# AutoGPTQ/AutoGPTQ

Hardware: AMD Instinct MI355X
Metric: int4 g128 QuantLinear fwd GB/s + tokens/s, Llama-7B shapes (higher is better)
Workload: dtype f16; 1 GPU; Llama-7B linear shapes (4096->4096 x4, 4096->11008 x2, 11008->4096) x 32 blocks = 224 layers, int4 g128 no act-order, M=1 rows per step, 128 launches/step in one hipGraph (q|k|v and gate|up of a block: one gptq_forward_multi launch each); layers=224, launches=128, parallelism=single

## Files before the change

### autogptq_amd/csrc/gemv_tiled_kernel.cuh

```cuda
#pragma once
#include <cstddef>

#include "gemv_shared.cuh"

namespace gptq {

struct TiledSeg {
    const void* bias;
    void* out;
    int N, col0;
};
struct PeerEpi {
    char* xbuf[2][GPTQ_PEER_MAX];
    unsigned* flags[GPTQ_PEER_MAX];
    unsigned* state;
    int world, rank;
    unsigned row_bytes, col_off_bytes, owners, pad_;
};
struct TiledParams {
    int blk_end[4];
    const void* x;
    int M, K;
    int chunks, chunks_per_split, ksplit, gu_shift, groups, xstride, waves;
    int pair_strips;
    const unsigned* tq[4];
    const void* cst[4];
    const int* perm[4];
    int xraw_off;
    int nseg, nsum;
    unsigned max_spins;
    TiledSeg seg[4];
    unsigned long long* gran;
    unsigned* epochs;
    unsigned* err;
    PeerEpi peer;
};
static_assert(offsetof(TiledParams, perm) == 128, "the entry batch of the decode-copy kernel is the first two cache lines of its arguments");

template <int BITS> struct TiledFmt;
template <> struct TiledFmt<4> { static constexpr int WPL = 4, KPL = 32, REC = 48, ZB = 1; };
template <> struct TiledFmt<8> { static constexpr int WPL = 4, KPL = 16, REC = 64, ZB = 2; };
template <> struct TiledFmt<3> { static constexpr int WPL = 3, KPL = 32, REC = 48, ZB = 1; };
template <> struct TiledFmt<2> { static constexpr int WPL = 2, KPL = 32, REC = 48, ZB = 1; };

#ifdef GPTQ_TILED_STAMPS
#define TILED_STAMP(i) (st_[i] = __builtin_amdgcn_s_memtime() | vz_)
#define TILED_STAMPS_OUT() stamps_out()
#define TILED_HOT_END() return
#else
#define TILED_HOT_END() __builtin_amdgcn_endpgm()
#define TILED_STAMP(i) ((void)0)
#define TILED_STAMPS_OUT() ((void)0)
#endif

template <int N_> struct WordsOf { typedef unsigned type __attribute__((ext_vector_type(N_))); };

template <int BITS, int MT, int U, typename T, int MAXW, int XM = 0, int ZM2 = 0>
__global__ void __launch_bounds__(MAXW * 64, MAXW == 16 ? 4 : 2) gemv_tiled_kernel(TiledParams p) {
#ifdef GPTQ_TILED_STAMPS
    unsigned long long st_[9] = {};
    unsigned vz_;
    asm volatile("v_mov_b32 %0, 0" : "=v"(vz_));
    st_[7] = __builtin_amdgcn_s_memrealtime() | vz_;
    TILED_STAMP(0);
    auto stamps_out = [&]() {
        st_[8] = __builtin_amdgcn_s_memrealtime() | vz_;
        unsigned long long* const dbg = p.gran;
        const int b = (int)blockIdx.x, nb = (int)gridDim.x;
        const int slot = b == 0 ? 0 : (b == 1 ? 1 : (b == nb / 2 ? 2 : (b == nb - 1 ? 3 : -1)));
        if (dbg != nullptr && p.ksplit == 1 && slot >= 0 && (threadIdx.x & 63) == 0) {
#pragma unroll
            for (int i = 0; i < 9; ++i) dbg[(slot * 16 + (int)(threadIdx.x >> 6)) * 16 + i] = st_[i];
        }
    };
#endif
    constexpr bool BF = std::is_same_v<T, bf16>;
    constexpr bool ACT = XM == 1, PEER = XM == 3;
    constexpr bool PAIR = XM == 4;
    constexpr bool MULTI = XM == 5 || XM == 6;
    constexpr int NSTR = PAIR ? 2 : (XM == 5 ? 4 : (XM == 6 ? 2 : 1));
    using F = TiledFmt<BITS>;
    constexpr int WPL = F::WPL, KPL = F::KPL, CKE = 4 * KPL, CHB = 64 * WPL * 4, REC = F::REC, NX = KPL / 8;
    constexpr int LKPL = KPL == 32 ? 5 : 4;
    typedef typename WordsOf<WPL>::type qvec;
    unsigned m_lo, m_hi, m_b, magic;
    asm("s_mov_b32 %0, 0x000f000f" : "=s"(m_lo));
    asm("s_mov_b32 %0, 0x00f000f0" : "=s"(m_hi));
    asm("s_mov_b32 %0, 0x00ff00ff" : "=s"(m_b));
    asm("v_mov_b32 %0, 0x64006400" : "=v"(magic));
    unsigned m2a, m2b, m2c, m2d, m2e;
    asm("s_mov_b32 %0, 0x00030003" : "=s"(m2a));
    asm("s_mov_b32 %0, 0x000c000c" : "=s"(m2b));
    asm("s_mov_b32 %0, 0x00300030" : "=s"(m2c));
    asm("s_mov_b32 %0, 0x00c000c0" : "=s"(m2d));
    asm("s_mov_b32 %0, 0x03000300" : "=s"(m2e));
    unsigned m3a, m3b, m3c;
    asm("s_mov_b32 %0, 0x00070007" : "=s"(m3a));
    asm("s_mov_b32 %0, 0x00380038" : "=s"(m3b));
    asm("s_mov_b32 %0, 0x01c001c0" : "=s"(m3c));
    extern __shared__ __attribute__((aligned(16))) char smem[];
    const int tid = threadIdx.x, lane = tid & 63;
    const int wave = __builtin_amdgcn_readfirstlane(tid >> 6);
    const int col = lane & 15, kb = lane >> 4;
    typedef unsigned u32x16 __attribute__((ext_vector_type(16)));
    typedef unsigned long long u64x8 __attribute__((ext_vector_type(8)));
    typedef unsigned long long u64x4 __attribute__((ext_vector_type(4)));
    static_assert(offsetof(TiledParams, x) == 16 && offsetof(TiledParams, M) == 24 && offsetof(TiledParams, chunks) == 32 && offsetof(TiledParams, pair_strips) == 60 &&
                  offsetof(TiledParams, tq) == 64 && offsetof(TiledParams, cst) == 96 && offsetof(TiledParams, perm) == 128 && offsetof(TiledParams, xraw_off) == 160, "the entry batch");
    u32x16 ha;
    u64x8 hb;
    [[maybe_unused]] u64x4 hp = {};
    [[maybe_unused]] int xraw_off = 0;
    {
        const auto kargs = __builtin_amdgcn_kernarg_segment_ptr();
        if constexpr (ACT)
            asm volatile("s_load_dwordx16 %0, %4, 0x0\n\ts_load_dwordx16 %1, %4, 0x40\n\ts_load_dwordx8 %2, %4, 0x80\n\ts_load_dword %3, %4, 0xa0\n\ts_waitcnt lgkmcnt(0)"
                         : "=&s"(ha), "=&s"(hb), "=&s"(hp), "=&s"(xraw_off) : "s"(kargs));
        else
            asm volatile("s_load_dwordx16 %0, %2, 0x0\n\ts_load_dwordx16 %1, %2, 0x40\n\ts_waitcnt lgkmcnt(0)" : "=&s"(ha), "=&s"(hb) : "s"(kargs));
    }
    const int be0 = (int)ha[0], be1 = (int)ha[1], be2 = (int)ha[2], Mrows = (int)ha[6], K = (int)ha[7], nchunks = (int)ha[8], cps = (int)ha[9], ksplit = (int)ha[10],
              gshift = (int)ha[11], G = (int)ha[12], xstride = (int)ha[13], W = (int)ha[14];
    [[maybe_unused]] const int hstrips = (int)ha[15];
    typedef __attribute__((address_space(1))) const char gchar;
    gchar* const xg = (gchar*)(((unsigned long long)ha[5] << 32) | ha[4]);
    int sidx = blockIdx.x, ks = 0, cb = 0, ce = nchunks, kbeg = 0, kend = K;
    if (__builtin_expect(ksplit != 1, 0)) {
        sidx = (int)blockIdx.x / ksplit; ks = (int)blockIdx.x - sidx * ksplit;
        cb = ks * cps; ce = min(cb + cps, nchunks);
        kbeg = cb * CKE; kend = min(ce * CKE, K);
    }
    unsigned long long tqs_ = hb[0], csts_ = hb[4];
    [[maybe_unused]] unsigned long long perm_ = hp[0];
    int sbase = 0, s = 0;
    if constexpr (ACT)
        asm("s_cmp_ge_i32 %[i], %[e0]\n\ts_cbranch_scc0 1f\n\t"
            "s_mov_b64 %[tq], %[tq1]\n\ts_mov_b64 %[cs], %[cs1]\n\ts_mov_b64 %[pm], %[pm1]\n\ts_mov_b32 %[sb], %[e0]\n\ts_mov_b32 %[s], 1\n\t"
            "s_cmp_ge_i32 %[i], %[e1]\n\ts_cselect_b64 %[tq], %[tq2], %[tq]\n\ts_cselect_b64 %[cs], %[cs2], %[cs]\n\ts_cselect_b64 %[pm], %[pm2], %[pm]\n\ts_cselect_b32 %[sb], %[e1], %[sb]\n\ts_cselect_b32 %[s], 2, %[s]\n\t"
            "s_cmp_ge_i32 %[i], %[e2]\n\ts_cselect_b64 %[tq], %[tq3], %[tq]\n\ts_cselect_b64 %[cs], %[cs3], %[cs]\n\ts_cselect_b64 %[pm], %[pm3], %[pm]\n\ts_cselect_b32 %[sb], %[e2], %[sb]\n\ts_cselect_b32 %[s], 3, %[s]\n"
            "1:"
            : [tq] "+&s"(tqs_), [cs] "+&s"(csts_), [pm] "+&s"(perm_), [sb] "+&s"(sbase), [s] "+&s"(s)
            : [i] "s"(sidx), [e0] "s"(be0), [e1] "s"(be1), [e2] "s"(be2), [tq1] "s"(hb[1]), [tq2] "s"(hb[2]), [tq3] "s"(hb[3]), [cs1] "s"(hb[5]), [cs2] "s"(hb[6]), [cs3] "s"(hb[7]),
              [pm1] "s"(hp[1]), [pm2] "s"(hp[2]), [pm3] "s"(hp[3])
            : "scc");
    else
        asm("s_cmp_ge_i32 %[i], %[e0]\n\ts_cbranch_scc0 1f\n\t"
            "s_mov_b64 %[tq], %[tq1]\n\ts_mov_b64 %[cs], %[cs1]\n\ts_mov_b32 %[sb], %[e0]\n\ts_mov_b32 %[s], 1\n\t"
            "s_cmp_ge_i32 %[i], %[e1]\n\ts_cselect_b64 %[tq], %[tq2], %[tq]\n\ts_cselect_b64 %[cs], %[cs2], %[cs]\n\ts_cselect_b32 %[sb], %[e1], %[sb]\n\ts_cselect_b32 %[s], 2, %[s]\n\t"
            "s_cmp_ge_i32 %[i], %[e2]\n\ts_cselect_b64 %[tq], %[tq3], %[tq]\n\ts_cselect_b64 %[cs], %[cs3], %[cs]\n\ts_cselect_b32 %[sb], %[e2], %[sb]\n\ts_cselect_b32 %[s], 3, %[s]\n"
            "1:"
            : [tq] "+&s"(tqs_), [cs] "+&s"(csts_), [sb] "+&s"(sbase), [s] "+&s"(s)
            : [i] "s"(sidx), [e0] "s"(be0), [e1] "s"(be1), [e2] "s"(be2), [tq1] "s"(hb[1]), [tq2] "s"(hb[2]), [tq3] "s"(hb[3]), [cs1] "s"(hb[5]), [cs2] "s"(hb[6]), [cs3] "s"(hb[7])
            : "scc");
    gchar* const tqs = (gchar*)tqs_;
    gchar* const csts = (gchar*)csts_;
    [[maybe_unused]] const int* const permp = (const int*)perm_;
    const int strip = sidx - sbase;
    const int Wh = NSTR == 4 ? (W >> 2) : (NSTR == 2 ? (W >> 1) : W);
    const int sel = NSTR == 1 ? 0 : (scalar_ge(wave, Wh) + (NSTR == 4 ? scalar_ge(wave, 2 * Wh) + scalar_ge(wave, 3 * Wh) : 0));
    const int wv = NSTR == 1 ? wave : wave - sel * Wh;
    const int strip_w = PAIR ? strip + sel * hstrips : (MULTI ? strip * NSTR + sel : strip);
    char* const xs = smem;
    char* const cs = smem + (size_t)MT * xstride;
    const unsigned crec = (unsigned)G * (unsigned)REC;
    const size_t cpad = ((size_t)crec + 15) & ~(size_t)15;
    float* const red = (float*)(cs + NSTR * cpad);
    gchar* const tb = tqs + (size_t)(unsigned)strip_w * ((unsigned)nchunks * (unsigned)CHB);
    gchar* const cg = csts + (size_t)(unsigned)(MULTI ? strip * NSTR : strip) * crec;
    const unsigned t_lane = (unsigned)lane * (WPL * 4u);
    auto stage_all = [&]() __attribute__((always_inline)) {
        const unsigned xs_lds = (unsigned)(size_t)(__attribute__((address_space(3))) char*)xs, cs_lds = (unsigned)(size_t)(__attribute__((address_space(3))) char*)cs;
        const int w64 = wave * 64, step = W * 64;
        gchar* xrow[MT];
        unsigned xdst[MT];
        if constexpr (XM == 0 || XM == 3 || XM == 4 || MULTI) {
#pragma unroll
            for (int m = 0; m < MT; ++m) {
                xrow[m] = xg + (unsigned)((m == 0 ? 0 : min(m, Mrows - 1)) * K + kbeg) * 2u;
                xdst[m] = xs_lds + m * xstride;
            }
            stage_rows<MT, false>(xrow, xdst, tid, w64, step, (kend - kbeg) >> 3);
        } else if constexpr (ACT) {
#pragma unroll
            for (int m = 0; m < MT; ++m) {
                xrow[m] = xg + (unsigned)((m == 0 ? 0 : min(m, Mrows - 1)) * K) * 2u;
                xdst[m] = xs_lds + (unsigned)xraw_off + m * (K * 2 + 16);
            }
            stage_rows<MT, false>(xrow, xdst, tid, w64, step, K >> 3);
        }
        const int cpieces = (int)(crec >> 4) * (MULTI ? NSTR : 1);
        if constexpr (PAIR) {
            gchar* const crow[2] = {cg, cg + (size_t)(unsigned)hstrips * crec};
            const unsigned cdst[2] = {cs_lds, cs_lds + (unsigned)cpad};
            stage_rows<2, true>(crow, cdst, tid, w64, step, cpieces);
        } else {
            gchar* const crow[1] = {cg};
            const unsigned cdst[1] = {cs_lds};
            stage_rows<1, true>(crow, cdst, tid, w64, step, cpieces);
        }
    };
#ifndef GPTQ_TILED_WEIGHTS_FIRST
    stage_all();
#endif
    typedef int i32x4 __attribute__((ext_vector_type(4)));
    i32x4 pa[2][2] = {};
    const int apieces = ACT ? (kend - kbeg) >> 3 : 0;
    if constexpr (ACT) {
        const int* const pg = permp + kbeg;
        if (tid < apieces) { pa[0][0] = *(const i32x4*)(pg + tid * 8); pa[0][1] = *(const i32x4*)(pg + tid * 8 + 4); }
        if (tid + W * 64 < apieces) { pa[1][0] = *(const i32x4*)(pg + (tid + W * 64) * 8); pa[1][1] = *(const i32x4*)(pg + (tid + W * 64) * 8 + 4); }
    }
    auto x_gather = [&]() {
        const int* const pg = permp + kbeg;
        const char* const xraw = smem + xraw_off;
        for (int pc0 = tid; pc0 < apieces; pc0 += 2 * W * 64) {
            const int pcb = pc0 + W * 64;
            const bool two = pcb < apieces;
            if (pc0 != tid) {
                pa[0][0] = *(const i32x4*)(pg + pc0 * 8); pa[0][1] = *(const i32x4*)(pg + pc0 * 8 + 4);
                if (two) { pa[1][0] = *(const i32x4*)(pg + pcb * 8); pa[1][1] = *(const i32x4*)(pg + pcb * 8 + 4); }
            }
#pragma unroll
            for (int m = 0; m < MT; ++m) {
                const unsigned short* xr = (const unsigned short*)(xraw + (size_t)m * (K * 2 + 16));
#pragma unroll
                for (int h = 0; h < 2; ++h) {
                    if (h == 1 && !two) break;
                    unsigned short v[8];
#pragma unroll
                    for (int i = 0; i < 8; ++i) v[i] = xr[pa[h][i >> 2][i & 3]];
                    u32x4 o;
#pragma unroll
                    for (int i = 0; i < 4; ++i) o[i] = (unsigned)v[2 * i] | ((unsigned)v[2 * i + 1] << 16);
                    *(u32x4*)(xs + (size_t)m * xstride + (size_t)(h ? pcb : pc0) * 16) = o;
                }
            }
        }
    };
#if defined(GPTQ_TILED_ZM)
    constexpr bool ZM = BITS == 4 && MT <= 4 && (GPTQ_TILED_ZM == 2 || (GPTQ_TILED_ZM == 1 && BF));
#else
    constexpr bool ZM = BITS == 4 && BF && (MT == 4 || (MT == 2 && ZM2 == 1));
#endif
#ifdef GPTQ_TILED_NO_XS
    constexpr bool XS = false;
#else
    constexpr bool XS = BF && BITS == 4 && MT <= 2 && !ZM;
#endif
    constexpr bool XC = BF && MT <= 2 && !XS && !ZM;
    using MM = std::conditional_t<XC, f16, T>;
    constexpr int ES = MT * 16 + 4;
    float* const xe = red + W * ES;
    auto x_to_f16 = [&]() {
        const int prow = (kend - kbeg) >> 3, total = prow * MT;
        for (int i0 = 0; i0 < total; i0 += W * 64) {
            const int idx = i0 + tid;
            const bool ok = idx < total;
            int m = 0, pc = ok ? idx : 0;
            if constexpr (MT > 1) { m = pc / prow; pc -= m * prow; }
            u32x4* const at = (u32x4*)(xs + (size_t)m * xstride + (size_t)pc * 16);
            u32x4 v = {0u, 0u, 0u, 0u};
            if (ok) v = *at;
            unsigned mx = 0u;
#pragma unroll
            for (int i = 0; i < 4; ++i) {
                const unsigned a = v[i] & 0x7fff7fffu;
                mx = max(mx, max(a & 0xffffu, a >> 16));
            }
            mx = max(mx, (unsigned)__shfl_xor((int)mx, 1, 64));
            if constexpr (NX == 4) mx = max(mx, (unsigned)__shfl_xor((int)mx, 2, 64));
            const int E = (int)((mx >> 7) & 0xffu);
            const int ms = min(max(268 - E, 1), 253);
            const float mult = __builtin_bit_cast(float, (unsigned)ms << 23);
#pragma unroll
            for (int i = 0; i < 4; ++i) {
                const float lo = __builtin_bit_cast(float, v[i] << 16) * mult, hi = __builtin_bit_cast(float, v[i] & 0xffff0000u) * mult;
                v[i] = __builtin_bit_cast(unsigned, __builtin_amdgcn_cvt_pkrtz(lo, hi));
            }
            if (ok) {
                *at = v;
                if ((pc & (NX - 1)) == 0) xe[(pc / NX) * 4 + m] = __builtin_bit_cast(float, (unsigned)(254 - ms) << 23);
            }
        }
        __syncthreads();
    };
    auto x_sums = [&]() {
        const int prow = (kend - kbeg) >> 3, total = prow * MT;
        for (int i0 = 0; i0 < total; i0 += W * 64) {
            const int idx = i0 + tid;
            const bool ok = idx < total;
            int m = 0, pc = ok ? idx : 0;
            if constexpr (MT > 1) { m = pc / prow; pc -= m * prow; }
            u32x4 v = {0u, 0u, 0u, 0u};
            if (ok) v = *(const u32x4*)(xs + (size_t)m * xstride + (size_t)pc * 16);
            float sm = 0.f;
#pragma unroll
            for (int i = 0; i < 4; ++i) sm += __builtin_bit_cast(float, v[i] << 16) + __builtin_bit_cast(float, v[i] & 0xffff0000u);
            sm += __shfl_xor(sm, 1, 64);
            if constexpr (NX == 4) sm += __shfl_xor(sm, 2, 64);
            if (ok && (pc & (NX - 1)) == 0) xe[(pc / NX) * 4 + m] = sm;
        }
        __syncthreads();
    };
    const char* const xl = xs + (size_t)min(lane & 3, MT - 1) * xstride + kb * (KPL * 2);
    const char* const xl2 = xs + (size_t)min(4 + (lane & 3), MT - 1) * xstride + kb * (KPL * 2);
    float acc[MT];
#pragma unroll
    for (int m = 0; m < MT; ++m) acc[m] = 0.f;
    const f16x2 k960 = {(f16)960.f, (f16)960.f}, k896 = {(f16)896.f, (f16)896.f}, k1008 = {(f16)1008.f, (f16)1008.f};
    const f16x2 r16 = {(f16)0.0625f, (f16)0.0625f}, r8 = {(f16)0.125f, (f16)0.125f}, r64 = {(f16)0.015625f, (f16)0.015625f};
    const f16x2 k768 = {(f16)768.f, (f16)768.f}, k1020 = {(f16)1020.f, (f16)1020.f}, r4 = {(f16)0.25f, (f16)0.25f}, r256 = {(f16)0.00390625f, (f16)0.00390625f};
    auto bits_of = [&](f16x2 hv) -> unsigned {
        if constexpr (BF && !XC) {
            const bf16x2 o = {(bf16)(float)hv[0], (bf16)(float)hv[1]};
            return __builtin_bit_cast(unsigned, o);
        } else {
            return __builtin_bit_cast(unsigned, hv);
        }
    };
    constexpr int E = MT * 16, NE = (MULTI ? NSTR : 1) * E;
    const int n_t = (MULTI ? strip * NSTR + tid / E : strip) * 16 + (tid & 15);
    float bv0 = 0.f, bv1 = 0.f;
    typedef __attribute__((address_space(1))) T gT;
    int N = 0;
    const void* biasp = nullptr;
    void* outp = nullptr;
    auto seg_request = [&]() __attribute__((always_inline)) {
        int sl = s;
        asm volatile("" : "+s"(sl) : : "memory");
        N = p.seg[sl].N; biasp = p.seg[sl].bias; outp = p.seg[sl].out;
    };
    auto seg_pin = [&]() __attribute__((always_inline)) { asm volatile("" : "+s"(N), "+s"(biasp), "+s"(outp)); };
    bool staged = false;
    for (int cbase = cb; cbase < ce; cbase += Wh * U) {
        const int c0 = cbase + wv * U;
        qvec q[U];
#pragma unroll
        for (int j = 0; j < U; ++j) q[j] = __builtin_nontemporal_load((const __attribute__((address_space(1))) qvec*)(tb + ((unsigned)min(c0 + j, ce - 1) * (unsigned)CHB + t_lane)));
        if (!staged) {
            TILED_STAMP(1);
            seg_request();
#ifdef GPTQ_TILED_WEIGHTS_FIRST
            stage_all();
            asm volatile("s_waitcnt vmcnt(0)" ::: "memory");
#else
            asm volatile("s_waitcnt vmcnt(%0)" ::"n"(U) : "memory");
#endif
            if constexpr (ACT) {
                __syncthreads();
                x_gather();
            }
            __syncthreads();
            if constexpr (XC) x_to_f16();
            if constexpr (XS) x_sums();
            seg_pin();
            if (biasp != nullptr && tid < NE && n_t < (PAIR ? N >> 1 : N)) {
                bv0 = DType<T>::to_f32(((const gT*)biasp)[n_t]);
                if constexpr (PAIR) bv1 = DType<T>::to_f32(((const gT*)biasp)[n_t + (N >> 1)]);
            }
            TILED_STAMP(2);
            staged = true;
        }
#ifdef GPTQ_TILED_STAMPS
        if (cbase + Wh * U >= ce) { asm volatile("s_waitcnt vmcnt(0)" ::: "memory"); TILED_STAMP(3); }
#endif
#pragma unroll
        for (int j = 0; j < U; ++j) {
            const int cc = min(c0 + j, ce - 1);
            const int k0 = cc * CKE + kb * KPL;
            const bool live = (c0 + j < ce) && (k0 < K);
            const int g = min(k0 >> LKPL >> gshift, G - 1);
            const char* cp = cs + (NSTR > 1 ? (size_t)sel * cpad : (size_t)0) + g * REC;
            const unsigned short sraw = *(const unsigned short*)(cp + col * 2);
            unsigned z;
            if constexpr (F::ZB == 1) z = *(const unsigned char*)(cp + 32 + col);
            else z = *(const unsigned short*)(cp + 32 + col * 2);
            u32x4 xa[NX];
#pragma unroll
            for (int w = 0; w < NX; ++w) xa[w] = *(const u32x4*)(xl + ((unsigned)(cc - cb) * (unsigned)(CKE * 2) + w * 16u));
            u32x4 xb[MT > 4 ? NX : 1];
            if constexpr (MT > 4) {
#pragma unroll
                for (int w = 0; w < NX; ++w) xb[w] = *(const u32x4*)(xl2 + ((unsigned)(cc - cb) * (unsigned)(CKE * 2) + w * 16u));
            }
            const f16x2 c1 = as_f16x2(z * 0x00010001u + 0xE400E400u);
            const qvec qv = q[j];
            f32x4 accg = {0.f, 0.f, 0.f, 0.f}, accg2 = {0.f, 0.f, 0.f, 0.f};
            auto mm = [&](int pc, int hf, unsigned b0, unsigned b1) __attribute__((always_inline)) {
                accg = Mma4<MM>::run(u32x2{xa[pc][hf * 2], xa[pc][hf * 2 + 1]}, u32x2{b0, b1}, accg);
                if constexpr (MT > 4) accg2 = Mma4<MM>::run(u32x2{xb[pc][hf * 2], xb[pc][hf * 2 + 1]}, u32x2{b0, b1}, accg2);
            };
            if constexpr (BITS == 4 && ZM) {
                unsigned mgz;
                asm("v_mov_b32 %0, %1" : "=v"(mgz) : "n"(BF ? 0x43004300 : 0x64006400));
                const unsigned nz = z * 0x00010001u + (BF ? 0xC300C300u : 0xE400E400u);
                f32x4 accz = {0.f, 0.f, 0.f, 0.f};
#pragma unroll
                for (int w = 0; w < 4; ++w) {
                    const unsigned qw = qv[w];
                    mm(w, 0, (qw & m_lo) | mgz, ((qw >> 4) & m_lo) | mgz);
                    mm(w, 1, ((qw >> 8) & m_lo) | mgz, ((qw >> 12) & m_lo) | mgz);
                    accz = Mma4<MM>::run(u32x2{xa[w][0], xa[w][1]}, u32x2{nz, nz}, accz);
                    accz = Mma4<MM>::run(u32x2{xa[w][2], xa[w][3]}, u32x2{nz, nz}, accz);
                }
                accg += accz;
            } else if constexpr (BITS == 4 && XS) {
                unsigned magicb;
                asm("v_mov_b32 %0, 0x43004300" : "=v"(magicb));
#pragma unroll
                for (int w = 0; w < 4; ++w) {
                    const unsigned qw = qv[w];
                    mm(w, 0, (qw & m_lo) | magicb, ((qw >> 4) & m_lo) | magicb);
                    mm(w, 1, ((qw >> 8) & m_lo) | magicb, ((qw >> 12) & m_lo) | magicb);
                }
            } else if constexpr (BITS == 4) {
                const f16x2 c2 = c1 + k960;
#pragma unroll
                for (int w = 0; w < 4; ++w) {
                    const unsigned qw = qv[w], q8 = qw >> 8;
                    const f16x2 h0 = as_f16x2((qw & m_lo) | magic) + c1;
                    const f16x2 h1 = as_f16x2((qw & m_hi) | magic) * r16 + c2;
                    const f16x2 h2 = as_f16x2((q8 & m_lo) | magic) + c1;
                    const f16x2 h3 = as_f16x2((q8 & m_hi) | magic) * r16 + c2;
                    mm(w, 0, bits_of(h0), bits_of(h1));
                    mm(w, 1, bits_of(h2), bits_of(h3));
                }
            } else if constexpr (BITS == 2) {
                const f16x2 c4 = c1 + k768, c16 = c1 + k960, c64 = c1 + k1008, c256 = c1 + k1020;
#pragma unroll
                for (int w = 0; w < 2; ++w) {
                    const unsigned t = qv[w], t10 = t >> 10;
                    const unsigned p0 = bits_of(as_f16x2((t & m2a) | magic) + c1);
                    const unsigned p1 = bits_of(as_f16x2((t & m2b) | magic) * r4 + c4);
                    const unsigned p2 = bits_of(as_f16x2((t & m2c) | magic) * r16 + c16);
                    const unsigned p3 = bits_of(as_f16x2((t & m2d) | magic) * r64 + c64);
                    const unsigned p4 = bits_of(as_f16x2((t & m2e) | magic) * r256 + c256);
                    const unsigned p5 = bits_of(as_f16x2((t10 & m2a) | magic) + c1);
                    const unsigned p6 = bits_of(as_f16x2((t10 & m2b) | magic) * r4 + c4);
                    const unsigned p7 = bits_of(as_f16x2((t10 & m2c) | magic) * r16 + c16);
                    mm(2 * w, 0, p0, p1);
                    mm(2 * w, 1, p2, p3);
                    mm(2 * w + 1, 0, p4, p5);
                    mm(2 * w + 1, 1, p6, p7);
                }
            } else if constexpr (BITS == 8) {
#pragma unroll
                for (int w = 0; w < 4; ++w) {
                    const unsigned qw = qv[w], q8 = qw >> 8;
                    const f16x2 h0 = as_f16x2((qw & m_b) | magic) + c1;
                    const f16x2 h1 = as_f16x2((q8 & m_b) | magic) + c1;
                    mm(w >> 1, w & 1, bits_of(h0), bits_of(h1));
                }
            } else {
                const f16x2 c3 = c1 + k896;
                const f16x2 c6 = c1 + k1008;
                unsigned pr[16];
#pragma unroll
                for (int w = 0; w < 3; ++w) {
                    const unsigned t = qv[w], t6 = t >> 6;
                    pr[5 * w + 0] = bits_of(as_f16x2((t & m3a) | magic) + c1);
                    pr[5 * w + 1] = bits_of(as_f16x2((t & m3b) | magic) * r8 + c3);
                    pr[5 * w + 2] = bits_of(as_f16x2((t & m3c) | magic) * r64 + c6);
                    pr[5 * w + 3] = bits_of(as_f16x2((t6 & m3b) | magic) * r8 + c3);
                    pr[5 * w + 4] = bits_of(as_f16x2((t6 & m3c) | magic) * r64 + c6);
                }
                const unsigned e = ((qv[0] >> 15) & 0x00010001u) | ((qv[1] >> 14) & 0x00020002u) | ((qv[2] >> 13) & 0x00040004u);
                pr[15] = bits_of(as_f16x2(e | magic) + c1);
#pragma unroll
                for (int i = 0; i < 8; ++i) mm(i >> 1, i & 1, pr[2 * i], pr[2 * i + 1]);
            }
            const float sc = DType<T>::to_f32(__builtin_bit_cast(T, sraw));
            if constexpr (XS) {
                const float* const xv = xe + ((cc - cb) * 4 + kb) * 4;
                const float zc = (float)(128u + z);
#pragma unroll
                for (int m = 0; m < MT; ++m) acc[m] = live ? fmaf(sc, fmaf(-zc, xv[m], accg[m]), acc[m]) : acc[m];
            } else if constexpr (XC) {
                const float* const xi = xe + ((cc - cb) * 4 + kb) * 4;
#pragma unroll
                for (int m = 0; m < MT; ++m) acc[m] = live ? fmaf(sc * xi[m], accg[m], acc[m]) : acc[m];
            } else {
#pragma unroll
                for (int m = 0; m < MT; ++m) acc[m] = live ? fmaf(sc, m < 4 ? accg[m] : accg2[m - 4], acc[m]) : acc[m];
            }
        }
    }
    TILED_STAMP(4);
#pragma unroll
    for (int m = 0; m < MT; ++m) acc[m] = kslot_sum_swap(acc[m]);
    if (__builtin_expect(!staged, 0)) {
        seg_request();
        seg_pin();
        __syncthreads();
    }
    gT* const outg = (gT*)outp;
    if (lane < 16) {
#pragma unroll
        for (int m = 0; m < MT; ++m) red[wave * ES + m * 16 + lane] = acc[m];
    }
    __syncthreads();
    TILED_STAMP(5);
    if constexpr (PAIR) {
        const int NH = N >> 1;
        if (tid < E) {
            const int m = tid >> 4;
            const float* const r = red + tid;
            float s0 = 0.f, s1 = 0.f;
            if (Wh == 4) { s0 = seq_sum<4, ES>(r); s1 = seq_sum<4, ES>(r + 4 * ES); }
            else if (MAXW == 16 && Wh == 8) { s0 = seq_sum<8, ES>(r); s1 = seq_sum<8, ES>(r + 8 * ES); }
            else if (Wh == 2) { s0 = seq_sum<2, ES>(r); s1 = seq_sum<2, ES>(r + 2 * ES); }
            else for (int w = 0; w < Wh; ++w) { s0 += r[w * ES]; s1 += r[(Wh + w) * ES]; }
            if (m < Mrows && n_t < NH) {
                if (biasp != nullptr) { s0 += bv0; s1 += bv1; }
                const float g = s0 / (1.f + __expf(-s0));
                outg[(size_t)m * NH + n_t] = DType<T>::from_f32(g * s1);
            }
        }
        TILED_STAMP(6);
        TILED_STAMPS_OUT();
        return;
    }
    if constexpr (MULTI) {
        const bool lean = (NE <= W * 64) & ((((MAXW == 16 ? 0x114u : 0x14u) >> (Wh & 31)) & 1u) != 0u);
        if (__builtin_expect(lean, 1)) {
            if (tid < NE) {
                const int s4 = tid / E, r = tid & (E - 1), m = r >> 4;
                float t;
                constexpr int WHOT = (XM == 6 && MT <= 2) ? 2 : 4;
                if (__builtin_expect(Wh == WHOT, 1)) t = seq_sum<WHOT, ES>(red + s4 * WHOT * ES + r);
                else if (Wh == 6 - WHOT) t = seq_sum<6 - WHOT, ES>(red + s4 * (6 - WHOT) * ES + r);
                else if constexpr (MAXW == 16) t = seq_sum<8, ES>(red + s4 * 8 * ES + r);
                else t = 0.f;
                if (m < Mrows && n_t < N) {
                    if (biasp != nullptr) t += bv0;
                    outg[(size_t)m * N + n_t] = DType<T>::from_f32(t);
                }
            }
            TILED_STAMP(6);
            TILED_STAMPS_OUT();
            TILED_HOT_END();
        }
        for (int e = tid; e < NSTR * MT * 16; e += W * 64) {
            const int s4 = e / (MT * 16), r = e - s4 * (MT * 16), m = r >> 4, c = r & 15, n = (strip * NSTR + s4) * 16 + c;
            float t = 0.f;
            for (int w = 0; w < Wh; ++w) t += red[(s4 * Wh + w) * ES + r];
            if (m < Mrows && n < N) {
                if (biasp) t += DType<T>::to_f32(((const T*)biasp)[n]);
                ((T*)outp)[(size_t)m * N + n] = DType<T>::from_f32(t);
            }
        }
        return;
    }
    if constexpr (!PEER) {
        const bool lean = (ksplit == 1) & ((((MAXW == 16 ? 0x10110u : 0x110u) >> (W & 31)) & 1u) != 0u);
        if (__builtin_expect(lean, 1)) {
            if (tid < E) {
                const int m = tid >> 4;
                const float* const r = red + tid;
                float t;
                constexpr int WHOT = MAXW == 16 ? 16 : 4;
                if (__builtin_expect(W == WHOT, 1)) t = tree_sum<WHOT, ES>(r);
                else if (MAXW == 8 || W == 8) t = tree_sum<8, ES>(r);
                else t = tree_sum<4, ES>(r);
                if (m < Mrows && n_t < N) {
                    if (biasp != nullptr) t += bv0;
                    outg[(size_t)m * N + n_t] = DType<T>::from_f32(t);
                }
            }
            TILED_STAMP(6);
            TILED_STAMPS_OUT();
            TILED_HOT_END();
        }
    }
    T* const stage = PEER ? (T*)xs : nullptr;
    const TiledSeg sg{biasp, outp, N, ksplit != 1 ? p.seg[s].col0 : 0};
    stream_finish<16, MT, T, TiledParams, TiledSeg>(p, sg, strip, sidx, ks, N, red, stage);
    if constexpr (PEER) if (ks == 0) {
        const int pworld = p.peer.world;
        __syncthreads();
        const unsigned e = __hip_atomic_load(p.peer.state, __ATOMIC_RELAXED, __HIP_MEMORY_SCOPE_AGENT) + 1u;
        if (tid < pworld * MT * 2) {
            const int r = tid / (MT * 2), m = (tid >> 1) % MT, q = tid & 1;
            if (m < Mrows) {
                const u32x4 v = *(const u32x4*)((const char*)stage + m * 32 + q * 16);
                char* const dst = p.peer.xbuf[e & 1u][r] + (size_t)m * p.peer.row_bytes + p.peer.col_off_bytes + (size_t)strip * 32 + q * 16;
                asm volatile("global_store_dwordx4 %0, %1, off sc0 sc1\n\ts_nop 1" ::"v"(dst), "v"(v) : "memory");
            }
        }
    }
}

template <int U, int XM> constexpr int tiled_maxw() { return (U == 2 || XM == 5) ? 16 : 8; }
int tiled_max_waves(int u, int nstr);
template <int BITS, int MT, int U, typename T, int XM>
static hipError_t launch_tiled_one(const TiledPlan& pl, const TiledParams& p, hipStream_t st) {
    constexpr int MAXW = tiled_maxw<U, XM>();
    if (pl.waves > MAXW) return hipErrorInvalidValue;
    if constexpr (BITS == 4 && MT == 2 && std::is_same_v<T, bf16> && (XM == 0 || XM == 1)) {
        if (pl.zm2) {
            hipLaunchKernelGGL((gemv_tiled_kernel<BITS, MT, U, T, MAXW, XM, 1>), dim3(pl.strips_total * pl.ksplit), dim3(pl.waves * 64), pl.lds_bytes, st, p);
            return hipGetLastError();
        }
    }
    hipLaunchKernelGGL((gemv_tiled_kernel<BITS, MT, U, T, MAXW, XM>), dim3(pl.strips_total * pl.ksplit), dim3(pl.waves * 64), pl.lds_bytes, st, p);
    return hipGetLastError();
}
template <int BITS, int MT, typename T, int XM>
static hipError_t launch_tiled_u(const TiledPlan& pl, const TiledParams& p, hipStream_t st) {
    switch (pl.u) {
        case 2: if constexpr (!(XM == 6 && MT <= 2)) return launch_tiled_one<BITS, MT, 2, T, XM>(pl, p, st); else return hipErrorInvalidValue;
        case 4: return launch_tiled_one<BITS, MT, 4, T, XM>(pl, p, st);
        default: return hipErrorInvalidValue;
    }
}
template <int BITS, typename T, int XM>
static hipError_t launch_tiled_mt(const TiledPlan& pl, const TiledParams& p, hipStream_t st) {
    constexpr bool LOW_OK = XM != 5 && (XM != 6 || BITS == 4);
    if constexpr (!LOW_OK) {
        if (pl.mt != 4 && pl.mt != 8) return hipErrorInvalidValue;
    }
    switch (pl.mt) {
        case 1: if constexpr (LOW_OK) return launch_tiled_u<BITS, 1, T, XM>(pl, p, st); else return hipErrorInvalidValue;
        case 2: if constexpr (LOW_OK) return launch_tiled_u<BITS, 2, T, XM>(pl, p, st); else return hipErrorInvalidValue;
        case 4: return launch_tiled_u<BITS, 4, T, XM>(pl, p, st);
        case 8: if constexpr (XM != 3 && XM != 4 && BITS != 2) return launch_tiled_u<BITS, 8, T, XM>(pl, p, st); else return hipErrorInvalidValue;
        default: return hipErrorInvalidValue;
    }
}
template <typename T, int XM>
static hipError_t launch_tiled_bits(const TiledPlan& pl, const TiledParams& p, hipStream_t st) {
    switch (pl.bits) {
        case 4: return launch_tiled_mt<4, T, XM>(pl, p, st);
        case 8: return launch_tiled_mt<8, T, XM>(pl, p, st);
        case 3: return launch_tiled_mt<3, T, XM>(pl, p, st);
        case 2:
            if constexpr (XM == 0 || XM == 1) { if (pl.mt <= 4) return launch_tiled_mt<2, T, XM>(pl, p, st); }
            return hipErrorInvalidValue;
        default: return hipErrorInvalidValue;
    }
}

template <int XM>
static hipError_t grant_tiled_lds() {
    hipError_t e = hipSuccess;
    auto grant = [&](auto kern) { hipError_t r = hipFuncSetAttribute((const void*)kern, hipFuncAttributeMaxDynamicSharedMemorySize, 160 * 1024); if (e == hipSuccess) e = r; };
    auto grant_mt = [&](auto mt) {
        constexpr int MT = decltype(mt)::value;
        auto grant_u = [&](auto bu, auto uu) {
            constexpr int B = decltype(bu)::value, U = decltype(uu)::value;
            constexpr int MAXW = tiled_maxw<U, XM>();
            grant(gemv_tiled_kernel<B, MT, U, f16, MAXW, XM>); grant(gemv_tiled_kernel<B, MT, U, bf16, MAXW, XM>);
            if constexpr (B == 4 && MT == 2 && (XM == 0 || XM == 1)) grant(gemv_tiled_kernel<B, MT, U, bf16, MAXW, XM, 1>);
        };
        using I2 = std::integral_constant<int, 2>; using I3 = std::integral_constant<int, 3>; using I4 = std::integral_constant<int, 4>; using I8 = std::integral_constant<int, 8>;
        grant_u(I4{}, I2{}); grant_u(I4{}, I4{});
        grant_u(I8{}, I2{}); grant_u(I8{}, I4{}); grant_u(I3{}, I2{}); grant_u(I3{}, I4{});
        if constexpr ((XM == 0 || XM == 1) && MT <= 4) { grant_u(I2{}, I2{}); grant_u(I2{}, I4{}); }
    };
    if constexpr (XM != 5 && XM != 6) { grant_mt(std::integral_constant<int, 1>{}); grant_mt(std::integral_constant<int, 2>{}); }
    if constexpr (XM == 6) {
        grant(gemv_tiled_kernel<4, 1, 4, f16, 8, 6>); grant(gemv_tiled_kernel<4, 1, 4, bf16, 8, 6>);
        grant(gemv_tiled_kernel<4, 2, 4, f16, 8, 6>); grant(gemv_tiled_kernel<4, 2, 4, bf16, 8, 6>);
    }
    grant_mt(std::integral_constant<int, 4>{});
    if constexpr (XM != 3 && XM != 4) grant_mt(std::integral_constant<int, 8>{});
    return e;
}

}
```

Before: 3745 GB/s.

## Software-pipeline weight loads with rolling prefetch across chunk iterations

The per-chunk dequant+MMA body is split into lambdas, and the main loop is restructured into a rolling register pipeline. Once chunk j has been consumed, the load for the matching chunk of the next iteration is issued right away, with sched_barriers pinning the order. This keeps global weight loads in flight during compute instead of waiting for all U loads at the top of each iteration. It costs ordering freedom for the scheduler, and the old loop stays available behind a macro.

```diff
diff --git a/autogptq_amd/csrc/gemv_tiled_kernel.cuh b/autogptq_amd/csrc/gemv_tiled_kernel.cuh
--- a/autogptq_amd/csrc/gemv_tiled_kernel.cuh
+++ b/autogptq_amd/csrc/gemv_tiled_kernel.cuh
@@ -332,159 +332,190 @@
     };
     auto seg_pin = [&]() __attribute__((always_inline)) { asm volatile("" : "+s"(N), "+s"(biasp), "+s"(outp)); };
     bool staged = false;
+    auto wload = [&](int c) __attribute__((always_inline)) -> qvec {
+        return __builtin_nontemporal_load((const __attribute__((address_space(1))) qvec*)(tb + ((unsigned)min(c, ce - 1) * (unsigned)CHB + t_lane)));
+    };
+    auto first_pass = [&]() __attribute__((always_inline)) {
+        TILED_STAMP(1);
+        seg_request();
+#ifdef GPTQ_TILED_WEIGHTS_FIRST
+        stage_all();
+        asm volatile("s_waitcnt vmcnt(0)" ::: "memory");
+#else
+        asm volatile("s_waitcnt vmcnt(%0)" ::"n"(U) : "memory");
+#endif
+        if constexpr (ACT) {
+            __syncthreads();
+            x_gather();
+        }
+        __syncthreads();
+        if constexpr (XC) x_to_f16();
+        if constexpr (XS) x_sums();
+        seg_pin();
+        if (biasp != nullptr && tid < NE && n_t < (PAIR ? N >> 1 : N)) {
+            bv0 = DType<T>::to_f32(((const gT*)biasp)[n_t]);
+            if constexpr (PAIR) bv1 = DType<T>::to_f32(((const gT*)biasp)[n_t + (N >> 1)]);
+        }
+        TILED_STAMP(2);
+        staged = true;
+    };
+    auto chunk = [&](const int cj, const qvec qv) __attribute__((always_inline)) {
+        const int cc = min(cj, ce - 1);
+        const int k0 = cc * CKE + kb * KPL;
+        const bool live = (cj < ce) && (k0 < K);
+        const int g = min(k0 >> LKPL >> gshift, G - 1);
+        const char* cp = cs + (NSTR > 1 ? (size_t)sel * cpad : (size_t)0) + g * REC;
+        const unsigned short sraw = *(const unsigned short*)(cp + col * 2);
+        unsigned z;
+        if constexpr (F::ZB == 1) z = *(const unsigned char*)(cp + 32 + col);
+        else z = *(const unsigned short*)(cp + 32 + col * 2);
+        u32x4 xa[NX];
+#pragma unroll
+        for (int w = 0; w < NX; ++w) xa[w] = *(const u32x4*)(xl + ((unsigned)(cc - cb) * (unsigned)(CKE * 2) + w * 16u));
+        u32x4 xb[MT > 4 ? NX : 1];
+        if constexpr (MT > 4) {
+#pragma unroll
+            for (int w = 0; w < NX; ++w) xb[w] = *(const u32x4*)(xl2 + ((unsigned)(cc - cb) * (unsigned)(CKE * 2) + w * 16u));
+        }
+        const f16x2 c1 = as_f16x2(z * 0x00010001u + 0xE400E400u);
+        f32x4 accg = {0.f, 0.f, 0.f, 0.f}, accg2 = {0.f, 0.f, 0.f, 0.f};
+        auto mm = [&](int pc, int hf, unsigned b0, unsigned b1) __attribute__((always_inline)) {
+            accg = Mma4<MM>::run(u32x2{xa[pc][hf * 2], xa[pc][hf * 2 + 1]}, u32x2{b0, b1}, accg);
+            if constexpr (MT > 4) accg2 = Mma4<MM>::run(u32x2{xb[pc][hf * 2], xb[pc][hf * 2 + 1]}, u32x2{b0, b1}, accg2);
+        };
+        if constexpr (BITS == 4 && ZM) {
+            unsigned mgz;
+            asm("v_mov_b32 %0, %1" : "=v"(mgz) : "n"(BF ? 0x43004300 : 0x64006400));
+            const unsigned nz = z * 0x00010001u + (BF ? 0xC300C300u : 0xE400E400u);
+            f32x4 accz = {0.f, 0.f, 0.f, 0.f};
+#pragma unroll
+            for (int w = 0; w < 4; ++w) {
+                const unsigned qw = qv[w];
+                mm(w, 0, (qw & m_lo) | mgz, ((qw >> 4) & m_lo) | mgz);
+                mm(w, 1, ((qw >> 8) & m_lo) | mgz, ((qw >> 12) & m_lo) | mgz);
+                accz = Mma4<MM>::run(u32x2{xa[w][0], xa[w][1]}, u32x2{nz, nz}, accz);
+                accz = Mma4<MM>::run(u32x2{xa[w][2], xa[w][3]}, u32x2{nz, nz}, accz);
+            }
+            accg += accz;
+        } else if constexpr (BITS == 4 && XS) {
+            unsigned magicb;
+            asm("v_mov_b32 %0, 0x43004300" : "=v"(magicb));
+#pragma unroll
+            for (int w = 0; w < 4; ++w) {
+                const unsigned qw = qv[w];
+                mm(w, 0, (qw & m_lo) | magicb, ((qw >> 4) & m_lo) | magicb);
+                mm(w, 1, ((qw >> 8) & m_lo) | magicb, ((qw >> 12) & m_lo) | magicb);
+            }
+        } else if constexpr (BITS == 4) {
+            const f16x2 c2 = c1 + k960;
+#pragma unroll
+            for (int w = 0; w < 4; ++w) {
+                const unsigned qw = qv[w], q8 = qw >> 8;
+                const f16x2 h0 = as_f16x2((qw & m_lo) | magic) + c1;
+                const f16x2 h1 = as_f16x2((qw & m_hi) | magic) * r16 + c2;
+                const f16x2 h2 = as_f16x2((q8 & m_lo) | magic) + c1;
+                const f16x2 h3 = as_f16x2((q8 & m_hi) | magic) * r16 + c2;
+                mm(w, 0, bits_of(h0), bits_of(h1));
+                mm(w, 1, bits_of(h2), bits_of(h3));
+            }
+        } else if constexpr (BITS == 2) {
+            const f16x2 c4 = c1 + k768, c16 = c1 + k960, c64 = c1 + k1008, c256 = c1 + k1020;
+#pragma unroll
+            for (int w = 0; w < 2; ++w) {
+                const unsigned t = qv[w], t10 = t >> 10;
+                const unsigned p0 = bits_of(as_f16x2((t & m2a) | magic) + c1);
+                const unsigned p1 = bits_of(as_f16x2((t & m2b) | magic) * r4 + c4);
+                const unsigned p2 = bits_of(as_f16x2((t & m2c) | magic) * r16 + c16);
+                const unsigned p3 = bits_of(as_f16x2((t & m2d) | magic) * r64 + c64);
+                const unsigned p4 = bits_of(as_f16x2((t & m2e) | magic) * r256 + c256);
+                const unsigned p5 = bits_of(as_f16x2((t10 & m2a) | magic) + c1);
+                const unsigned p6 = bits_of(as_f16x2((t10 & m2b) | magic) * r4 + c4);
+                const unsigned p7 = bits_of(as_f16x2((t10 & m2c) | magic) * r16 + c16);
+                mm(2 * w, 0, p0, p1);
+                mm(2 * w, 1, p2, p3);
+                mm(2 * w + 1, 0, p4, p5);
+                mm(2 * w + 1, 1, p6, p7);
+            }
+        } else if constexpr (BITS == 8) {
+#pragma unroll
+            for (int w = 0; w < 4; ++w) {
+                const unsigned qw = qv[w], q8 = qw >> 8;
+                const f16x2 h0 = as_f16x2((qw & m_b) | magic) + c1;
+                const f16x2 h1 = as_f16x2((q8 & m_b) | magic) + c1;
+                mm(w >> 1, w & 1, bits_of(h0), bits_of(h1));
+            }
+        } else {
+            const f16x2 c3 = c1 + k896;
+            const f16x2 c6 = c1 + k1008;
+            unsigned pr[16];
+#pragma unroll
+            for (int w = 0; w < 3; ++w) {
+                const unsigned t = qv[w], t6 = t >> 6;
+                pr[5 * w + 0] = bits_of(as_f16x2((t & m3a) | magic) + c1);
+                pr[5 * w + 1] = bits_of(as_f16x2((t & m3b) | magic) * r8 + c3);
+                pr[5 * w + 2] = bits_of(as_f16x2((t & m3c) | magic) * r64 + c6);
+                pr[5 * w + 3] = bits_of(as_f16x2((t6 & m3b) | magic) * r8 + c3);
+                pr[5 * w + 4] = bits_of(as_f16x2((t6 & m3c) | magic) * r64 + c6);
+            }
+            const unsigned e = ((qv[0] >> 15) & 0x00010001u) | ((qv[1] >> 14) & 0x00020002u) | ((qv[2] >> 13) & 0x00040004u);
+            pr[15] = bits_of(as_f16x2(e | magic) + c1);
+#pragma unroll
+            for (int i = 0; i < 8; ++i) mm(i >> 1, i & 1, pr[2 * i], pr[2 * i + 1]);
+        }
+        unsigned sr_ = sraw;
+        asm volatile("" : "+v"(sr_));
+        const float sc = DType<T>::to_f32(__builtin_bit_cast(T, (unsigned short)sr_));
+        if constexpr (XS) {
+            const float* const xv = xe + ((cc - cb) * 4 + kb) * 4;
+            const float zc = (float)(128u + z);
+#pragma unroll
+            for (int m = 0; m < MT; ++m) acc[m] = live ? fmaf(sc, fmaf(-zc, xv[m], accg[m]), acc[m]) : acc[m];
+        } else if constexpr (XC) {
+            const float* const xi = xe + ((cc - cb) * 4 + kb) * 4;
+#pragma unroll
+            for (int m = 0; m < MT; ++m) acc[m] = live ? fmaf(sc * xi[m], accg[m], acc[m]) : acc[m];
+        } else {
+#pragma unroll
+            for (int m = 0; m < MT; ++m) acc[m] = live ? fmaf(sc, m < 4 ? accg[m] : accg2[m - 4], acc[m]) : acc[m];
+        }
+    };
+#ifdef GPTQ_TILED_NO_ROLL
     for (int cbase = cb; cbase < ce; cbase += Wh * U) {
         const int c0 = cbase + wv * U;
         qvec q[U];
 #pragma unroll
-        for (int j = 0; j < U; ++j) q[j] = __builtin_nontemporal_load((const __attribute__((address_space(1))) qvec*)(tb + ((unsigned)min(c0 + j, ce - 1) * (unsigned)CHB + t_lane)));
-        if (!staged) {
-            TILED_STAMP(1);
-            seg_request();
-#ifdef GPTQ_TILED_WEIGHTS_FIRST
-            stage_all();
-            asm volatile("s_waitcnt vmcnt(0)" ::: "memory");
-#else
-            asm volatile("s_waitcnt vmcnt(%0)" ::"n"(U) : "memory");
-#endif
-            if constexpr (ACT) {
-                __syncthreads();
-                x_gather();
-            }
-            __syncthreads();
-            if constexpr (XC) x_to_f16();
-            if constexpr (XS) x_sums();
-            seg_pin();
-            if (biasp != nullptr && tid < NE && n_t < (PAIR ? N >> 1 : N)) {
-                bv0 = DType<T>::to_f32(((const gT*)biasp)[n_t]);
-                if constexpr (PAIR) bv1 = DType<T>::to_f32(((const gT*)biasp)[n_t + (N >> 1)]);
-            }
-            TILED_STAMP(2);
-            staged = true;
-        }
+        for (int j = 0; j < U; ++j) q[j] = wload(c0 + j);
+        if (!staged) first_pass();
 #ifdef GPTQ_TILED_STAMPS
         if (cbase + Wh * U >= ce) { asm volatile("s_waitcnt vmcnt(0)" ::: "memory"); TILED_STAMP(3); }
 #endif
 #pragma unroll
-        for (int j = 0; j < U; ++j) {
-            const int cc = min(c0 + j, ce - 1);
-            const int k0 = cc * CKE + kb * KPL;
-            const bool live = (c0 + j < ce) && (k0 < K);
-            const int g = min(k0 >> LKPL >> gshift, G - 1);
-            const char* cp = cs + (NSTR > 1 ? (size_t)sel * cpad : (size_t)0) + g * REC;
-            const unsigned short sraw = *(const unsigned short*)(cp + col * 2);
-            unsigned z;
-            if constexpr (F::ZB == 1) z = *(const unsigned char*)(cp + 32 + col);
-            else z = *(const unsigned short*)(cp + 32 + col * 2);
-            u32x4 xa[NX];
-#pragma unroll
-            for (int w = 0; w < NX; ++w) xa[w] = *(const u32x4*)(xl + ((unsigned)(cc - cb) * (unsigned)(CKE * 2) + w * 16u));
-            u32x4 xb[MT > 4 ? NX : 1];
-            if constexpr (MT > 4) {
-#pragma unroll
-                for (int w = 0; w < NX; ++w) xb[w] = *(const u32x4*)(xl2 + ((unsigned)(cc - cb) * (unsigned)(CKE * 2) + w * 16u));
-            }
-            const f16x2 c1 = as_f16x2(z * 0x00010001u + 0xE400E400u);
-            const qvec qv = q[j];
-            f32x4 accg = {0.f, 0.f, 0.f, 0.f}, accg2 = {0.f, 0.f, 0.f, 0.f};
-            auto mm = [&](int pc, int hf, unsigned b0, unsigned b1) __attribute__((always_inline)) {
-                accg = Mma4<MM>::run(u32x2{xa[pc][hf * 2], xa[pc][hf * 2 + 1]}, u32x2{b0, b1}, accg);
-                if constexpr (MT > 4) accg2 = Mma4<MM>::run(u32x2{xb[pc][hf * 2], xb[pc][hf * 2 + 1]}, u32x2{b0, b1}, accg2);
-            };
-            if constexpr (BITS == 4 && ZM) {
-                unsigned mgz;
-                asm("v_mov_b32 %0, %1" : "=v"(mgz) : "n"(BF ? 0x43004300 : 0x64006400));
-                const unsigned nz = z * 0x00010001u + (BF ? 0xC300C300u : 0xE400E400u);
-                f32x4 accz = {0.f, 0.f, 0.f, 0.f};
-#pragma unroll
-                for (int w = 0; w < 4; ++w) {
-                    const unsigned qw = qv[w];
-                    mm(w, 0, (qw & m_lo) | mgz, ((qw >> 4) & m_lo) | mgz);
-                    mm(w, 1, ((qw >> 8) & m_lo) | mgz, ((qw >> 12) & m_lo) | mgz);
-                    accz = Mma4<MM>::run(u32x2{xa[w][0], xa[w][1]}, u32x2{nz, nz}, accz);
-                    accz = Mma4<MM>::run(u32x2{xa[w][2], xa[w][3]}, u32x2{nz, nz}, accz);
-                }
-                accg += accz;
-            } else if constexpr (BITS == 4 && XS) {
-                unsigned magicb;
-                asm("v_mov_b32 %0, 0x43004300" : "=v"(magicb));
-#pragma unroll
-                for (int w = 0; w < 4; ++w) {
-                    const unsigned qw = qv[w];
-                    mm(w, 0, (qw & m_lo) | magicb, ((qw >> 4) & m_lo) | magicb);
-                    mm(w, 1, ((qw >> 8) & m_lo) | magicb, ((qw >> 12) & m_lo) | magicb);
-                }
-            } else if constexpr (BITS == 4) {
-                const f16x2 c2 = c1 + k960;
-#pragma unroll
-                for (int w = 0; w < 4; ++w) {
-                    const unsigned qw = qv[w], q8 = qw >> 8;
-                    const f16x2 h0 = as_f16x2((qw & m_lo) | magic) + c1;
-                    const f16x2 h1 = as_f16x2((qw & m_hi) | magic) * r16 + c2;
-                    const f16x2 h2 = as_f16x2((q8 & m_lo) | magic) + c1;
-                    const f16x2 h3 = as_f16x2((q8 & m_hi) | magic) * r16 + c2;
-                    mm(w, 0, bits_of(h0), bits_of(h1));
-                    mm(w, 1, bits_of(h2), bits_of(h3));
-                }
-            } else if constexpr (BITS == 2) {
-                const f16x2 c4 = c1 + k768, c16 = c1 + k960, c64 = c1 + k1008, c256 = c1 + k1020;
-#pragma unroll
-                for (int w = 0; w < 2; ++w) {
-                    const unsigned t = qv[w], t10 = t >> 10;
-                    const unsigned p0 = bits_of(as_f16x2((t & m2a) | magic) + c1);
-                    const unsigned p1 = bits_of(as_f16x2((t & m2b) | magic) * r4 + c4);
-                    const unsigned p2 = bits_of(as_f16x2((t & m2c) | magic) * r16 + c16);
-                    const unsigned p3 = bits_of(as_f16x2((t & m2d) | magic) * r64 + c64);
-                    const unsigned p4 = bits_of(as_f16x2((t & m2e) | magic) * r256 + c256);
-                    const unsigned p5 = bits_of(as_f16x2((t10 & m2a) | magic) + c1);
-                    const unsigned p6 = bits_of(as_f16x2((t10 & m2b) | magic) * r4 + c4);
-                    const unsigned p7 = bits_of(as_f16x2((t10 & m2c) | magic) * r16 + c16);
-                    mm(2 * w, 0, p0, p1);
-                    mm(2 * w, 1, p2, p3);
-                    mm(2 * w + 1, 0, p4, p5);
-                    mm(2 * w + 1, 1, p6, p7);
-                }
-            } else if constexpr (BITS == 8) {
-#pragma unroll
-                for (int w = 0; w < 4; ++w) {
-                    const unsigned qw = qv[w], q8 = qw >> 8;
-                    const f16x2 h0 = as_f16x2((qw & m_b) | magic) + c1;
-                    const f16x2 h1 = as_f16x2((q8 & m_b) | magic) + c1;
-                    mm(w >> 1, w & 1, bits_of(h0), bits_of(h1));
-                }
-            } else {
-                const f16x2 c3 = c1 + k896;
-                const f16x2 c6 = c1 + k1008;
-                unsigned pr[16];
-#pragma unroll
-                for (int w = 0; w < 3; ++w) {
-                    const unsigned t = qv[w], t6 = t >> 6;
-                    pr[5 * w + 0] = bits_of(as_f16x2((t & m3a) | magic) + c1);
-                    pr[5 * w + 1] = bits_of(as_f16x2((t & m3b) | magic) * r8 + c3);
-                    pr[5 * w + 2] = bits_of(as_f16x2((t & m3c) | magic) * r64 + c6);
-                    pr[5 * w + 3] = bits_of(as_f16x2((t6 & m3b) | magic) * r8 + c3);
-                    pr[5 * w + 4] = bits_of(as_f16x2((t6 & m3c) | magic) * r64 + c6);
-                }
-                const unsigned e = ((qv[0] >> 15) & 0x00010001u) | ((qv[1] >> 14) & 0x00020002u) | ((qv[2] >> 13) & 0x00040004u);
-                pr[15] = bits_of(as_f16x2(e | magic) + c1);
-#pragma unroll
-                for (int i = 0; i < 8; ++i) mm(i >> 1, i & 1, pr[2 * i], pr[2 * i + 1]);
-            }
-            const float sc = DType<T>::to_f32(__builtin_bit_cast(T, sraw));
-            if constexpr (XS) {
-                const float* const xv = xe + ((cc - cb) * 4 + kb) * 4;
-                const float zc = (float)(128u + z);
-#pragma unroll
-                for (int m = 0; m < MT; ++m) acc[m] = live ? fmaf(sc, fmaf(-zc, xv[m], accg[m]), acc[m]) : acc[m];
-            } else if constexpr (XC) {
-                const float* const xi = xe + ((cc - cb) * 4 + kb) * 4;
-#pragma unroll
-                for (int m = 0; m < MT; ++m) acc[m] = live ? fmaf(sc * xi[m], accg[m], acc[m]) : acc[m];
-            } else {
-#pragma unroll
-                for (int m = 0; m < MT; ++m) acc[m] = live ? fmaf(sc, m < 4 ? accg[m] : accg2[m - 4], acc[m]) : acc[m];
-            }
-        }
-    }
+        for (int j = 0; j < U; ++j) chunk(c0 + j, q[j]);
+    }
+#else
+    if (cb < ce) {
+        int c0 = cb + wv * U;
+        qvec q[U];
+#pragma unroll
+        for (int j = 0; j < U; ++j) q[j] = wload(c0 + j);
+        first_pass();
+        for (int cn = c0 + Wh * U; cn < ce; cn += Wh * U) {
+#pragma unroll
+            for (int j = 0; j < U; ++j) {
+                chunk(c0 + j, q[j]);
+                __builtin_amdgcn_sched_barrier(0);
+                q[j] = wload(cn + j);
+                __builtin_amdgcn_sched_barrier(0);
+            }
+            c0 = cn;
+        }
+#ifdef GPTQ_TILED_STAMPS
+        asm volatile("s_waitcnt vmcnt(0)" ::: "memory"); TILED_STAMP(3);
+#endif
+#pragma unroll
+        for (int j = 0; j < U; ++j) chunk(c0 + j, q[j]);
+    }
+#endif
     TILED_STAMP(4);
 #pragma unroll
     for (int m = 0; m < MT; ++m) acc[m] = kslot_sum_swap(acc[m]);
```

New measurement: 3843 GB/s (median of 6 runs). 2.6% higher.
